# LLNL/parelag

Measured on NVIDIA B200. Metric: vcycle_dofs_per_s, higher is better.
Workload: dtype f64

## Files before the change

include/parelag_b200.h:

```cpp
#ifndef PARELAG_B200_H
#define PARELAG_B200_H

#include <stddef.h>
#include <stdint.h>

#ifdef __cplusplus
extern "C" {
#endif

typedef struct pe_ctx pe_ctx;
typedef struct pe_mat pe_mat;
typedef struct pe_vec pe_vec;
typedef struct pe_smoother pe_smoother;
typedef struct pe_graph pe_graph;

typedef struct pe_parcsr_host {
    int64_t global_num_rows, global_num_cols;
    int64_t first_row_index, first_col_diag;
    int32_t num_rows;
    int32_t num_cols_diag;
    int32_t num_cols_offd;
    const int32_t *diag_i, *diag_j;
    const double *diag_data;
    const int32_t *offd_i, *offd_j;
// ... 17 lines not shown
int pe_ctx_timer_start(pe_ctx *ctx);
int pe_ctx_timer_stop(pe_ctx *ctx, float *ms);
int pe_ctx_profile(pe_ctx *ctx, int enable);
int pe_ctx_profile_get(pe_ctx *ctx, int kernel_id, int64_t *count, double *total_ms, double *total_bytes);
enum { PE_TUNE_SELL_MIN_ROWS = 0, PE_TUNE_SELL_GROUP = 1, PE_TUNE_PDL = 2, PE_TUNE_GATHER_KEEP_PCT = 3, PE_TUNE_P2P_HALO = 4,
       PE_TUNE_FUSED_GS_MAX_MB = 5, PE_TUNE_GS_SLABS = 6, PE_TUNE_LOCAL_SMEM_BYTES = 7, PE_TUNE_COUNT = 8 };
int pe_set_tuning(int key, int value);
int pe_get_tuning(int key);
enum { PE_VARIANT_SPMV_SELL = 0, PE_VARIANT_SPMV_STREAM = 1, PE_VARIANT_SPMV_VECTOR = 2,
       PE_VARIANT_SPGEMM_SYM_T128 = 3, PE_VARIANT_SPGEMM_SYM_T1024 = 4, PE_VARIANT_SPGEMM_SYM_T8192 = 5, PE_VARIANT_SPGEMM_SYM_GMEM = 6,
       PE_VARIANT_SPGEMM_NUM_T128 = 7, PE_VARIANT_SPGEMM_NUM_T1024 = 8, PE_VARIANT_SPGEMM_NUM_T8192 = 9, PE_VARIANT_SPGEMM_NUM_GMEM = 10,
       PE_VARIANT_RELAX_TPR_1 = 11, PE_VARIANT_RELAX_TPR_2 = 12, PE_VARIANT_RELAX_TPR_4 = 13, PE_VARIANT_RELAX_TPR_8 = 14,
       PE_VARIANT_RELAX_TPR_16 = 15, PE_VARIANT_RELAX_TPR_32 = 16,
       PE_VARIANT_TRACES_SMEM = 17, PE_VARIANT_TRACES_GMEM = 18, PE_VARIANT_EXT_SMEM = 19, PE_VARIANT_EXT_GMEM = 20,
       PE_VARIANT_EXT_SPLIT_SMEM = 21, PE_VARIANT_TRACES_GMEM_REUSE = 22, PE_VARIANT_EXT_GMEM_REUSE = 23,
       PE_VARIANT_COUNT = 24 };
int pe_variant_counts(int64_t *out, int n, int reset);
int pe_ctx_flush_l2(pe_ctx *ctx);

int pe_graph_begin(pe_ctx *ctx);
int pe_graph_end(pe_ctx *ctx, pe_graph **out);
int pe_graph_launch(pe_ctx *ctx, pe_graph *g);
int pe_graph_free(pe_graph *g);

typedef struct pe_program pe_program;
int pe_program_begin(pe_ctx *ctx);
int pe_program_end(pe_ctx *ctx, pe_program **out);
int pe_program_launch(pe_ctx *ctx, pe_program *p);
int pe_program_free(pe_program *p);
int pe_program_info(const pe_program *p, int32_t *nops, double *algorithmic_bytes);
int pe_program_profile(pe_ctx *ctx, pe_program *p, int32_t *op_types, double *op_usec, double *op_bytes);
// ... 78 lines not shown
```

parelag_b200/capi.py:

```python
import ctypes as C
import os
import re

import numpy as np

_HERE = os.path.dirname(os.path.abspath(__file__))
LIB_PATH = os.path.join(_HERE, "lib", "libparelag_b200.so")
HEADER_PATHS = [os.path.join(os.path.dirname(_HERE), "include", "parelag_b200_local.h"),
                os.path.join(os.path.dirname(_HERE), "include", "parelag_b200.h"),
                os.path.join(os.path.dirname(_HERE), "include", "parelag_b200_api.h")]

_lib = None


class PEError(RuntimeError):
    pass


class ParCSRHost(C.Structure):
    _fields_ = [
        ("global_num_rows", C.c_int64), ("global_num_cols", C.c_int64),
        ("first_row_index", C.c_int64), ("first_col_diag", C.c_int64),
        ("num_rows", C.c_int32), ("num_cols_diag", C.c_int32), ("num_cols_offd", C.c_int32),
        ("diag_i", C.c_void_p), ("diag_j", C.c_void_p), ("diag_data", C.c_void_p),
# ... 110 lines not shown

def get_tuning(key):
    return lib().pe_get_tuning(key)


REPLAY_DIRECT = 0
REPLAY_GRAPH = 1
REPLAY_PROGRAM = 2
REPLAY_MODE_NAMES = {REPLAY_DIRECT: "direct", REPLAY_GRAPH: "graph", REPLAY_PROGRAM: "program"}

VARIANT_SLOTS = ("SPMV_SELL", "SPMV_STREAM", "SPMV_VECTOR",
                 "SPGEMM_SYM_T128", "SPGEMM_SYM_T1024", "SPGEMM_SYM_T8192", "SPGEMM_SYM_GMEM",
                 "SPGEMM_NUM_T128", "SPGEMM_NUM_T1024", "SPGEMM_NUM_T8192", "SPGEMM_NUM_GMEM",
                 "RELAX_TPR_1", "RELAX_TPR_2", "RELAX_TPR_4", "RELAX_TPR_8", "RELAX_TPR_16", "RELAX_TPR_32",
                 "TRACES_SMEM", "TRACES_GMEM", "EXT_SMEM", "EXT_GMEM",
                 "EXT_SPLIT_SMEM", "TRACES_GMEM_REUSE", "EXT_GMEM_REUSE")
(SPMV_SELL, SPMV_STREAM, SPMV_VECTOR,
 SPGEMM_SYM_T128, SPGEMM_SYM_T1024, SPGEMM_SYM_T8192, SPGEMM_SYM_GMEM,
 SPGEMM_NUM_T128, SPGEMM_NUM_T1024, SPGEMM_NUM_T8192, SPGEMM_NUM_GMEM,
 RELAX_TPR_1, RELAX_TPR_2, RELAX_TPR_4, RELAX_TPR_8, RELAX_TPR_16, RELAX_TPR_32,
 TRACES_SMEM, TRACES_GMEM, EXT_SMEM, EXT_GMEM,
 EXT_SPLIT_SMEM, TRACES_GMEM_REUSE, EXT_GMEM_REUSE) = range(len(VARIANT_SLOTS))


def variant_counts(reset=False):
    out = np.zeros(len(VARIANT_SLOTS), dtype=np.int64)
    _chk(lib().pe_variant_counts(_ptr(out), len(VARIANT_SLOTS), 1 if reset else 0))
    return out


def nccl_unique_id():
    buf = C.create_string_buffer(128)
    _chk(lib().pe_nccl_get_unique_id(buf))
    return buf.raw


class Vec:
# ... 222 lines not shown
```

parelag_b200/csrc/pe_core.cuh:

```cuda
#pragma once
#include <cuda_runtime.h>
#include <stdint.h>
#include <memory>
#include <string>
#include <vector>
#include "../../include/parelag_b200.h"

#define PE_SM_COUNT 148

void pe_set_error(const std::string &msg);

#define PE_CUDA(call)                                                              \
    do {                                                                           \
        cudaError_t e_ = (call);                                                   \
        if (e_ != cudaSuccess) {                                                   \
            pe_set_error(std::string(#call) + " failed: " + cudaGetErrorString(e_) \
                         + " at " + __FILE__ + ":" + std::to_string(__LINE__));    \
            return 1;                                                              \
        }                                                                          \
    } while (0)

#define PE_CHECK(cond, msg)                                     \
    do {                                                        \
        if (!(cond)) {                                          \
// ... 6 lines not shown
    do {                          \
        int rc_ = (expr);         \
        if (rc_) return rc_;      \
    } while (0)

#define PE_LAUNCHED(ctx)                                     \
    do {                                                     \
        (ctx)->launches++;                                   \
        if ((ctx)->rec) pe_rec_fail((ctx), __FILE__, __LINE__); \
        PE_CUDA(cudaPeekAtLastError());                      \
    } while (0)

enum PeOpType : int32_t {
    PE_OP_SELL_SPMV = 1, PE_OP_SELL_GS, PE_OP_CSR_SPMV, PE_OP_PERM_IN, PE_OP_PERM_OUT, PE_OP_AXPBY, PE_OP_ADD3,
    PE_OP_FILL, PE_OP_COPY, PE_OP_SCALE, PE_OP_MUL, PE_OP_DOT, PE_OP_DOT_FIN, PE_OP_AXPY_DEV, PE_OP_XPBY_DEV,
    PE_OP_PCG_STEP
};
struct PeOp {
    int32_t type, i0, i1, i2, i3, i4, i5, flags;
    int64_t n;
    double a, b;
    const void *p[9];
};
struct pe_recorder {
    std::vector<PeOp> ops;
    std::vector<double> bytes;
    bool failed = false;
    std::string why;
};
struct pe_ctx;
void pe_rec_fail(pe_ctx *ctx, const char *file, int line);
// ... 60 lines not shown
    }
    return cudaLaunchKernelEx(&cfg, kern, KArgs(args)...);
}
#endif
int pe_prof_begin(pe_ctx *ctx, int id, double bytes);
int pe_prof_end(pe_ctx *ctx);
#define PE_MAX_PARTIALS 4096

struct DevSELL {
    int32_t nslices = 0, nrows = 0;
    int32_t wmax = 0;
    int64_t nstored = 0;
    int32_t *soff = nullptr;
    int32_t *J = nullptr;
    double *A = nullptr;
};

struct DevCSR {
    int32_t nrows = 0, ncols = 0;
    int64_t nnz = 0;
    int32_t *I = nullptr, *J = nullptr;
    double *A = nullptr;
    int32_t *rb = nullptr;
    int32_t nrb = 0;
    DevSELL *sell = nullptr;
    int sell_state = 0;
};
void pe_sell_free(DevSELL &m);
int pe_sell_build(pe_ctx *ctx, const DevCSR &diag, const DevCSR *offd, const int32_t *rowmap_d, int32_t nslices,
                  const int32_t *colpos_d, int32_t ext_base, DevSELL &out,
                  std::vector<int32_t> *soff_host = nullptr);
int pe_sell_for_spmv(pe_ctx *ctx, DevCSR &m);
void pe_mat_values_changed(struct pe_mat *A);
int pe_launch_sell_spmv(pe_ctx *ctx, const DevSELL &S, double alpha, const double *x, double beta,
                        const double *yin, double *yout);
int pe_launch_sell_gs(pe_ctx *ctx, const DevSELL &S, int s0, int s1, int wmax, int ext_base, const double *f, double *u,
                      const double *uext, const double *l1, uint64_t pol_gather);
int pe_make_gather_policy(pe_ctx *ctx, int keep_pct, uint64_t *pol);
int pe_launch_perm_in(pe_ctx *ctx, int n, const int *pos, const double *b, const double *x, double *fp, double *up);
int pe_launch_perm_out(pe_ctx *ctx, int n, const int *pos, const double *up, double *x);
#define PE_STREAM_NNZ 2048
#define PE_STREAM_CAP 2560
#define PE_STREAM_MAXROW 512
int pe_build_row_blocks(pe_ctx *ctx, DevCSR &m, const std::vector<int32_t> *forced_breaks);
int devcsr_alloc(DevCSR &m, int32_t nrows, int32_t ncols, int64_t nnz);
void devcsr_free(DevCSR &m);

struct pe_vec {
    pe_ctx *ctx;
    int64_t n;
    double *d;
    bool view = false;
};

struct pe_mat {
// ... 54 lines not shown
```

parelag_b200/csrc/pe_prog.cu:

```cuda
#include "pe_core.cuh"
#include "pe_stream.cuh"
#include <cstring>

#define PROG_THREADS 1024
#define PROG_WARPS (PROG_THREADS / 32)

struct pe_program {
    pe_ctx *ctx = nullptr;
    PeOp *ops_d = nullptr;
    int nops = 0, grid = 0;
    unsigned long long *bar_d = nullptr;
    unsigned long long epoch = 0;
    unsigned long long *ts_d = nullptr;
    std::vector<int32_t> types;
    std::vector<double> bytes;
    double total_bytes = 0.0;
};

__device__ __forceinline__ unsigned long long ld_acquire_u64(const unsigned long long *p)
{
    unsigned long long v;
    asm volatile("ld.acquire.gpu.global.u64 %0, [%1];" : "=l"(v) : "l"(p) : "memory");
    return v;
}
__device__ __forceinline__ unsigned long long globaltimer_ns()
{
    unsigned long long t;
    asm volatile("mov.u64 %0, %globaltimer;" : "=l"(t));
    return t;
}

__device__ __noinline__ void op_sell_spmv(const PeOp &o, int gw, int W, int lane)
{
    const int nslices = o.i0, nrows = o.i1;
    const int *soff = (const int *)o.p[0], *J = (const int *)o.p[1];
    const double *A = (const double *)o.p[2], *x = (const double *)o.p[3], *yin = (const double *)o.p[4];
    double *yout = (double *)o.p[5];
    const double alpha = o.a, beta = o.b;
    const uint64_t pol = l2_evict_first_policy();
    for (int s = gw; s < nslices; s += W)
    {
        const int o0 = __ldg(soff + s), w = __ldg(soff + s + 1) - o0;
        const int *j = J + (int64_t)o0 * 32 + lane;
        const double *a = A + (int64_t)o0 * 32 + lane;
        double acc = 0.0;
        int q = 0;
        for (; q + 4 <= w; q += 4)
        {
            const int c0 = ld_stream_s32(j + (q + 0) * 32, pol), c1 = ld_stream_s32(j + (q + 1) * 32, pol);
            const int c2 = ld_stream_s32(j + (q + 2) * 32, pol), c3 = ld_stream_s32(j + (q + 3) * 32, pol);
            const double a0 = ld_stream_f64(a + (q + 0) * 32, pol), a1 = ld_stream_f64(a + (q + 1) * 32, pol);
            const double a2 = ld_stream_f64(a + (q + 2) * 32, pol), a3 = ld_stream_f64(a + (q + 3) * 32, pol);
            const double x0 = __ldcg(x + c0), x1 = __ldcg(x + c1), x2 = __ldcg(x + c2), x3 = __ldcg(x + c3);
            acc += a0 * x0; acc += a1 * x1; acc += a2 * x2; acc += a3 * x3;
        }
        for (; q < w; ++q) acc += ld_stream_f64(a + q * 32, pol) * __ldcg(x + ld_stream_s32(j + q * 32, pol));
        const int row = s * 32 + lane;
        if (row < nrows)
        {
            double v = alpha * acc;
            if (beta != 0.0) v += beta * __ldcg(yin + row);
            yout[row] = v;
        }
    }
}

__device__ __noinline__ void op_sell_gs(const PeOp &o, int gw, int W, int lane)
{
    const int s0 = o.i0, s1 = o.i1, ext_base = o.i2;
    const int *soff = (const int *)o.p[0], *J = (const int *)o.p[1];
    const double *A = (const double *)o.p[2], *f = (const double *)o.p[3];
    double *u = (double *)o.p[4];
    const double *uext = (const double *)o.p[5], *l1 = (const double *)o.p[6];
    const uint64_t pol = l2_evict_first_policy();
#define PE_GATHER(c) ((uext && (c) >= ext_base) ? __ldcg(uext + ((c) - ext_base)) : __ldcg(u + (c)))
    for (int s = s0 + gw; s < s1; s += W)
    {
        const int o0 = __ldg(soff + s), w = __ldg(soff + s + 1) - o0;
        const int *j = J + (int64_t)o0 * 32 + lane;
// ... 70 lines not shown
    }
}

__device__ __noinline__ void op_elementwise(const PeOp &o, int64_t gt, int64_t T)
{
    const int64_t n = o.n;
    const double a = o.a, b = o.b;
    switch (o.type)
    {
    case PE_OP_PERM_IN:
    {
        const int *pos = (const int *)o.p[0];
        const double *bv = (const double *)o.p[1], *x = (const double *)o.p[2];
        double *fp = (double *)o.p[3], *up = (double *)o.p[4];
        for (int64_t i = gt; i < n; i += T) { const int p = __ldg(pos + i); fp[p] = __ldcg(bv + i); up[p] = x ? __ldcg(x + i) : 0.0; }
        break;
    }
    case PE_OP_PERM_OUT:
    {
        const int *pos = (const int *)o.p[0];
        const double *up = (const double *)o.p[1];
        double *x = (double *)o.p[2];
        for (int64_t i = gt; i < n; i += T) x[i] = __ldcg(up + __ldg(pos + i));
        break;
    }
    case PE_OP_AXPBY:
    {
        const double *x = (const double *)o.p[0];
        double *y = (double *)o.p[1];
        if (b == 0.0) { for (int64_t i = gt; i < n; i += T) y[i] = a * __ldcg(x + i); }
// ... 248 lines not shown
```

parelag_b200/csrc/pe_relax.cu:

```cuda
#include "pe_core.cuh"
#include "pe_stream.cuh"
#include <algorithm>
#include <cmath>
#include <cstring>

struct pe_smoother {
    pe_ctx *ctx = nullptr;
    pe_mat *A = nullptr;
    int type = 2, sweeps = 1, cheby_order = 2, ordering = 0;
    double weight = 1.0, omega = 1.0, cheby_fraction = 0.3;
    double *l1_d = nullptr;
    double *v_d = nullptr, *w_d = nullptr, *z_d = nullptr, *r_d = nullptr;
    int32_t nsets = 0;
    std::vector<int32_t> set_starts;
    std::vector<int32_t> order;
    int32_t *perm_d = nullptr;
    DevCSR P;
    uint8_t *before_d = nullptr;
    int tpr = 8;
    std::vector<int> set_pI;
    std::vector<int> set_rb;
    int pI_at(int k) const { for (size_t c = 0; c < set_starts.size(); ++c) if (set_starts[c] == k) return set_pI[c]; return 0; }
    bool use_sell = false;
    DevSELL S;
// ... 889 lines not shown
extern "C" int pe_smoother_apply(pe_smoother *s, const pe_vec *b, pe_vec *x, int iterative_mode)
{
    pe_ctx *ctx = s->ctx;
    pe_mat *A = s->A;
    int n = A->diag.nrows;
    PE_CHECK(b->n == n && x->n == n, "pe_smoother_apply: size mismatch");
    cudaStream_t st = ctx->stream;
    if (s->use_sell)
    {
        const bool ghosts = A->offd.nnz > 0;
        for (int sweep = 0; sweep < s->sweeps; ++sweep)
        {
            const bool zero_guess = !iterative_mode && sweep == 0;
            PE_TRY(sweep_halo(A, x->d, zero_guess));
            if (s->fused && !ctx->rec) { PE_TRY(launch_fused_sweep(s, b->d, x->d, zero_guess)); continue; }
            PE_TRY(pe_launch_perm_in(ctx, n, s->pos_d, b->d, zero_guess ? nullptr : x->d, s->fp_d, s->up_d));
            for (int pass = 0; pass < 2; ++pass)
                for (int cc = (pass == 1 && s->skip_turn) ? 1 : 0; cc < s->nsets; ++cc)
                {
                    const int c = pass == 0 ? cc : s->nsets - 1 - cc;
                    if (s->slice_starts[c + 1] == s->slice_starts[c]) continue;
                    PE_TRY(pe_prof_begin(ctx, s->set_bytes[c] >= 64e6 ? 1 : 3, s->set_bytes[c]));
                    PE_TRY(pe_launch_sell_gs(ctx, s->S, s->slice_starts[c], s->slice_starts[c + 1], s->set_wmax[c], s->npad, s->fp_d, s->up_d,
                                             ghosts ? A->x_ext_d : nullptr, s->l1p_d, s->pol_gather));
                    PE_TRY(pe_prof_end(ctx));
                }
            PE_TRY(pe_launch_perm_out(ctx, n, s->pos_d, s->up_d, x->d));
        }
        return 0;
    }
    if (!iterative_mode) PE_CUDA(cudaMemsetAsync(x->d, 0, sizeof(double) * (size_t)n, st));
    const int *oI = A->offd.nnz > 0 ? A->offd.I : nullptr;
    for (int sweep = 0; sweep < s->sweeps; ++sweep) {
        if (s->type == 0 || s->type == 1 || s->type == 5) {
            PE_TRY(sweep_halo(A, x->d, !iterative_mode && sweep == 0));
            int tpr = A->tpr;
// ... 68 lines not shown
```

parelag_b200/csrc/pe_sell.cu:

```cuda
#include "pe_core.cuh"
#include "pe_stream.cuh"
#include <cub/cub.cuh>
#include <algorithm>

__device__ __forceinline__ int sell_src_row(const int *rowmap, int k, int nrows_src)
{
    if (rowmap) return rowmap[k];
    return k < nrows_src ? k : -1;
}

__global__ void k_sell_widths(int nslices, int nrows_src, const int *__restrict__ rowmap,
                              const int *__restrict__ dI, const int *__restrict__ oI, int *w)
{
    const int s = (blockIdx.x * blockDim.x + threadIdx.x) >> 5, lane = threadIdx.x & 31;
    if (s >= nslices) return;
    const int r = sell_src_row(rowmap, s * 32 + lane, nrows_src);
    int len = 0;
    if (r >= 0) { len = dI[r + 1] - dI[r]; if (oI) len += oI[r + 1] - oI[r]; }
    len = __reduce_max_sync(0xffffffffu, len);
    if (lane == 0) { w[s + 1] = len; if (s == 0) w[0] = 0; }
}

__global__ void k_sell_fill(int nslices, int nrows_src, const int *__restrict__ rowmap,
                            const int *__restrict__ colpos, int ext_base,
// ... 16 lines not shown
        }
        if (oI) for (int t = oI[r]; t < oI[r + 1]; ++t, ++q, p += 32)
        {
            last = ext_base + oJ[t];
            J[p] = last; A[p] = oA[t];
        }
    }
    for (; q < w; ++q, p += 32) { J[p] = last; A[p] = 0.0; }
}

void pe_sell_free(DevSELL &m)
{
    if (m.soff) cudaFree(m.soff);
    if (m.J) cudaFree(m.J);
    if (m.A) cudaFree(m.A);
    m = DevSELL();
}

int pe_sell_build(pe_ctx *ctx, const DevCSR &diag, const DevCSR *offd, const int32_t *rowmap_d, int32_t nslices,
                  const int32_t *colpos_d, int32_t ext_base, DevSELL &out, std::vector<int32_t> *soff_host)
{
    cudaStream_t st = ctx->stream;
    if (!rowmap_d) nslices = (diag.nrows + 31) / 32;
    out = DevSELL();
    out.nslices = nslices;
    out.nrows = diag.nrows;
    PE_CUDA(cudaMalloc(&out.soff, sizeof(int32_t) * (size_t)(nslices + 1)));
    if (nslices == 0) { PE_CUDA(cudaMemsetAsync(out.soff, 0, sizeof(int32_t), st)); return 0; }
    const int *oI = (offd && offd->nnz > 0) ? offd->I : nullptr;
    const int grid = pe_grid_for((int64_t)nslices * 32, 256);
// ... 12 lines not shown
    out.wmax = 0;
    for (int32_t k = 0; k < nslices; ++k) out.wmax = std::max(out.wmax, soff_h[k + 1] - soff_h[k]);
    if (soff_host) soff_host->swap(soff_h);
    out.nstored = (int64_t)total * 32;
    PE_CUDA(cudaMalloc(&out.J, sizeof(int32_t) * (size_t)(out.nstored > 0 ? out.nstored : 1)));
    PE_CUDA(cudaMalloc(&out.A, sizeof(double) * (size_t)(out.nstored > 0 ? out.nstored : 1)));
    if (out.nstored > 0)
    {
        k_sell_fill<<<grid, 256, 0, st>>>(nslices, diag.nrows, rowmap_d, colpos_d, ext_base, diag.I, diag.J, diag.A,
                                          oI, oI ? offd->J : nullptr, oI ? offd->A : nullptr, out.soff, out.J, out.A);
        PE_LAUNCHED(ctx);
    }
    return 0;
}

int pe_sell_for_spmv(pe_ctx *ctx, DevCSR &m)
{
    if (m.sell_state != 0) return 0;
    m.sell_state = -1;
    if (m.nnz == 0 || m.nrows == 0) return 0;
    DevSELL *s = new DevSELL();
    int rc = pe_sell_build(ctx, m, nullptr, nullptr, 0, nullptr, 0, *s);
    if (rc) { delete s; return rc; }
    if ((double)s->nstored > 1.25 * (double)m.nnz) { pe_sell_free(*s); delete s; return 0; }
    m.sell = s;
    m.sell_state = 1;
    return 0;
}

template <int G, bool PRO = false>
__device__ __forceinline__ void sell_load_group(const int *j, const double *a, int q, int w, uint64_t pol,
                                                int (&c)[G], double (&v)[G])
{
#pragma unroll
    for (int k = 0; k < G; ++k)
        if (q + k < w)
        {
            c[k] = PRO ? ld_stream_s32_pro(j + (q + k) * 32, pol) : ld_stream_s32(j + (q + k) * 32, pol);
            v[k] = PRO ? ld_stream_f64_pro(a + (q + k) * 32, pol) : ld_stream_f64(a + (q + k) * 32, pol);
        }
}

template <int G>
__device__ __forceinline__ void sell_pin_group_then_wait(const int (&c)[G], const double (&v)[G], int w)
{
    int t = 0;
#pragma unroll
    for (int k = 0; k < G; ++k) if (k < w) t ^= c[k] ^ __double2hiint(v[k]) ^ __double2loint(v[k]);
    if (t == 0x5bd1e995) pdl_trigger();
    pdl_wait();
}

template <int G, bool SINGLE>
__global__ void __launch_bounds__(256, ((SINGLE || G <= 4) ? 4 : 2))
k_sell_spmv(int nslices, int nrows, const int *__restrict__ soff, const int *__restrict__ J,
            const double *__restrict__ A, const double *x, double alpha, double beta,
            const double *yin, double *yout)
{
    pdl_trigger();
    const int s = (blockIdx.x * blockDim.x + threadIdx.x) >> 5, lane = threadIdx.x & 31;
    if (s >= nslices) { pdl_wait(); return; }
    const int o0 = ld_nc_s32_pro(soff + s), w = ld_nc_s32_pro(soff + s + 1) - o0;
    const int *j = J + (int64_t)o0 * 32 + lane;
    const double *a = A + (int64_t)o0 * 32 + lane;
    const uint64_t pol = l2_evict_first_policy();
    double acc = 0.0;
    int c[G]; double v[G];
    sell_load_group<G, true>(j, a, 0, w, pol, c, v);
    sell_pin_group_then_wait<G>(c, v, w);
    const int row = s * 32 + lane;
    const double yv = (beta != 0.0 && row < nrows) ? yin[row] : 0.0;
    for (int q = 0; q < w; q += G)
    {
        double xv[G], b[G];
#pragma unroll
        for (int k = 0; k < G; ++k) if (q + k < w) { xv[k] = x[c[k]]; b[k] = v[k]; }
        if (!SINGLE && q + G < w) sell_load_group<G>(j, a, q + G, w, pol, c, v);
#pragma unroll
        for (int k = 0; k < G; ++k) if (q + k < w) acc = __fma_rn(b[k], xv[k], acc);
// ... 47 lines not shown
    else if (wmax <= 4) G = 4;
    else if (wmax <= 8) G = 8;
    else if (wmax <= 12) G = 12;
    else if (wmax <= 24) G = 8;
    else G = 4;
    single = wmax <= G;
}

int pe_launch_sell_spmv(pe_ctx *ctx, const DevSELL &S, double alpha, const double *x, double beta,
                        const double *yin, double *yout)
{
    if (S.nslices == 0) return 0;
    if (ctx->rec)
    {
        PeOp o = pe_op(PE_OP_SELL_SPMV); o.i0 = S.nslices; o.i1 = S.nrows; o.a = alpha; o.b = beta;
        o.p[0] = S.soff; o.p[1] = S.J; o.p[2] = S.A; o.p[3] = x; o.p[4] = yin; o.p[5] = yout;
        pe_rec_push(ctx, o, -1.0);
        return 0;
    }
    const int grid = pe_grid_for((int64_t)S.nslices * 32, 256);
    int G; bool single;
    sell_pick_group(S.wmax, G, single);
#define PE_SPMV(GG, SS) PE_CUDA(pe_launch_k(ctx, k_sell_spmv<GG, SS>, grid, 256, S.nslices, S.nrows, S.soff, S.J, S.A, x, alpha, beta, yin, yout))
    if (G == 4) { if (single) PE_SPMV(4, true); else PE_SPMV(4, false); }
    else if (G == 8) { if (single) PE_SPMV(8, true); else PE_SPMV(8, false); }
    else { if (single) PE_SPMV(12, true); else PE_SPMV(12, false); }
#undef PE_SPMV
    PE_LAUNCHED(ctx);
    return 0;
}

template <int G, bool SINGLE, bool OFFD>
__global__ void __launch_bounds__(256, ((SINGLE || G <= 4) ? 4 : 2))
k_sell_gs(int s0, int s1, const int *__restrict__ soff, const int *__restrict__ J, const double *__restrict__ A,
          int ext_base, const double *f, double *u, const double *uext,
          const double *__restrict__ l1, uint64_t pol_u)
{
    pdl_trigger();
    const int s = s0 + ((blockIdx.x * blockDim.x + threadIdx.x) >> 5), lane = threadIdx.x & 31;
    if (s >= s1) { pdl_wait(); return; }
    const int o0 = ld_nc_s32_pro(soff + s), w = ld_nc_s32_pro(soff + s + 1) - o0;
    const int *j = J + (int64_t)o0 * 32 + lane;
// ... 66 lines not shown
    if (i < n) x[i] = up[p];
}
int pe_launch_perm_in(pe_ctx *ctx, int n, const int *pos, const double *b, const double *x, double *fp, double *up)
{
    if (n == 0) return 0;
    if (ctx->rec)
    {
        PeOp o = pe_op(PE_OP_PERM_IN); o.n = n; o.p[0] = pos; o.p[1] = b; o.p[2] = x; o.p[3] = fp; o.p[4] = up;
        pe_rec_push(ctx, o, 0.0);
        return 0;
    }
    PE_CUDA(pe_launch_k(ctx, k_sell_perm_in, pe_grid_for(n, 256), 256, n, pos, b, x, fp, up));
    PE_LAUNCHED(ctx);
    return 0;
}
int pe_launch_perm_out(pe_ctx *ctx, int n, const int *pos, const double *up, double *x)
{
    if (n == 0) return 0;
    if (ctx->rec)
    {
        PeOp o = pe_op(PE_OP_PERM_OUT); o.n = n; o.p[0] = pos; o.p[1] = up; o.p[2] = x;
        pe_rec_push(ctx, o, 0.0);
        return 0;
    }
    PE_CUDA(pe_launch_k(ctx, k_sell_perm_out, pe_grid_for(n, 256), 256, n, pos, up, x));
    PE_LAUNCHED(ctx);
    return 0;
}
```

parelag_b200/csrc/pe_spmv.cu:

```cuda
#include "pe_core.cuh"
#include <cub/cub.cuh>

__device__ __forceinline__ double ld_stream_f64(const double *p)
{
    double v;
    asm volatile("ld.global.nc.L1::no_allocate.f64 %0, [%1];" : "=d"(v) : "l"(p));
    return v;
}
__device__ __forceinline__ int ld_stream_s32(const int *p)
{
    int v;
    asm volatile("ld.global.nc.L1::no_allocate.s32 %0, [%1];" : "=r"(v) : "l"(p));
    return v;
}

template <int TPR>
__global__ void __launch_bounds__(256)
k_spmv(int n, const int *__restrict__ dI, const int *__restrict__ dJ, const double *__restrict__ dA,
       const int *__restrict__ oI, const int *__restrict__ oJ, const double *__restrict__ oA,
       const double *x, const double *xext,
       double alpha, double beta, const double *yin, double *yout)
{
    pdl_trigger();
    const int lane = threadIdx.x & (TPR - 1);
// ... 62 lines not shown
}

int pe_launch_spmv(pe_ctx *ctx, const DevCSR &diag, const DevCSR *offd, int tpr,
                   double alpha, const double *x, const double *xext,
                   double beta, const double *yin, double *yout)
{
    int n = diag.nrows;
    if (n == 0) return 0;
    const int *oI = nullptr, *oJ = nullptr;
    const double *oA = nullptr;
    if (offd && offd->nnz > 0) { oI = offd->I; oJ = offd->J; oA = offd->A; }
    if (!oI && diag.sell_state == 0) PE_TRY(pe_sell_for_spmv(ctx, const_cast<DevCSR &>(diag)));
    if (!oI && diag.sell)
    {
        pe_variant_add(PE_VARIANT_SPMV_SELL, n);
        PE_TRY(pe_prof_begin(ctx, 0, 12.0 * (double)diag.nnz + 4.0 * (n + 1) + 8.0 * diag.ncols + 8.0 * n + (beta != 0.0 ? 8.0 * n : 0.0)));
        PE_TRY(pe_launch_sell_spmv(ctx, *diag.sell, alpha, x, beta, yin, yout));
        PE_TRY(pe_prof_end(ctx));
        return 0;
    }
    if (ctx->rec && !oI)
    {
        pe_variant_add(PE_VARIANT_SPMV_VECTOR, n);
        PeOp o = pe_op(PE_OP_CSR_SPMV); o.i0 = n; o.i1 = pe_choose_tpr(diag.nnz, n); o.a = alpha; o.b = beta;
        o.p[0] = diag.I; o.p[1] = diag.J; o.p[2] = diag.A; o.p[3] = x; o.p[4] = yin; o.p[5] = yout;
        pe_rec_push(ctx, o, 12.0 * (double)diag.nnz + 4.0 * (n + 1) + 8.0 * diag.ncols + 8.0 * n + (beta != 0.0 ? 8.0 * n : 0.0));
        return 0;
    }
    if (!oI && diag.nrb == 0 && diag.nnz > 0) PE_TRY(pe_build_row_blocks(ctx, const_cast<DevCSR &>(diag), nullptr));
    if (!oI && diag.nrb > 0)
    {
// ... 203 lines not shown
```

parelag_b200/csrc/pe_stream.cuh:

```cuda
#pragma once
#include <stdint.h>
#include "../../include/parelag_b200.h"

__device__ __forceinline__ uint64_t l2_evict_first_policy()
{
    uint64_t pol;
    asm("createpolicy.fractional.L2::evict_first.b64 %0, 1.0;" : "=l"(pol));
    return pol;
}
__device__ __forceinline__ double ld_stream_f64(const double *p, uint64_t pol)
{
    double v;
    asm("ld.global.nc.L1::no_allocate.L2::cache_hint.f64 %0, [%1], %2;" : "=d"(v) : "l"(p), "l"(pol));
    return v;
}
__device__ __forceinline__ int ld_stream_s32(const int *p, uint64_t pol)
{
    int v;
    asm("ld.global.nc.L1::no_allocate.L2::cache_hint.s32 %0, [%1], %2;" : "=r"(v) : "l"(p), "l"(pol));
    return v;
}

__device__ __forceinline__ double ld_stream_f64_pro(const double *p, uint64_t pol)
{
    double v;
    asm volatile("ld.global.nc.L1::no_allocate.L2::cache_hint.f64 %0, [%1], %2;" : "=d"(v) : "l"(p), "l"(pol));
    return v;
}
__device__ __forceinline__ int ld_stream_s32_pro(const int *p, uint64_t pol)
{
    int v;
    asm volatile("ld.global.nc.L1::no_allocate.L2::cache_hint.s32 %0, [%1], %2;" : "=r"(v) : "l"(p), "l"(pol));
    return v;
}
__device__ __forceinline__ int ld_nc_s32_pro(const int *p)
{
    int v;
    asm volatile("ld.global.nc.s32 %0, [%1];" : "=r"(v) : "l"(p));
    return v;
}
__device__ __forceinline__ double ld_nc_f64_pro(const double *p)
{
    double v;
    asm volatile("ld.global.nc.f64 %0, [%1];" : "=d"(v) : "l"(p));
    return v;
}

__device__ __forceinline__ void pe_pcg_scalar_step_dev(double *s, int phase, int iter, int max_iter, double rel, double abs_tol)
// ... 47 lines not shown
```

parelag_b200/src/parelag_solvers.hpp:

```cpp
#pragma once
#include <algorithm>
#include <cctype>
#include <cmath>
#include <cstdio>
#include "parelag_core.hpp"
#include "parelag_sequence.hpp"
#include "parelag_block.hpp"

namespace parelag
{

namespace mg_utils
{
inline void ComputeResidual(const mfem::Operator &A, const mfem::Vector &x, const mfem::Vector &b, mfem::Vector &r)
{
    auto A_hyp = dynamic_cast<const mfem::HypreParMatrix *>(&A);
    if (!A_hyp) { ComputeResidualGeneric(A, x, b, r); return; }
    r.SetSize(b.Size());
    PE_CALL(pe_residual(Device::Get(), A_hyp->Handle(), x.Read(), b.Read(), r.Write()));
}
}

inline bool SolverCaptureSafe(const mfem::Solver *s)
{
// ... 97 lines not shown
    {
        PARELAG_ASSERT(A_); PARELAG_ASSERT(D_op_); PARELAG_ASSERT(PrimarySolver_); PARELAG_ASSERT(AuxiliarySolver_);
        AuxB_.SetSize(D_op_->Width());
        AuxX_.SetSize(D_op_->Width());
        PrimaryVec_.SetSize(A_->Height());
    }
    void Mult(const mfem::Vector &B, mfem::Vector &X) const override
    {
        if (this->IsPreconditioner()) X = 0.0;
        PARELAG_ASSERT(PrimarySolver_->iterative_mode);
        PrimarySolver_->Mult(B, X);
        mg_utils::ComputeResidual(*A_, X, B, PrimaryVec_);
        D_op_->MultTranspose(PrimaryVec_, AuxB_);
        PARELAG_ASSERT(!AuxiliarySolver_->iterative_mode);
        AuxiliarySolver_->Mult(AuxB_, AuxX_);
        D_op_->Mult(AuxX_, PrimaryVec_);
        X += PrimaryVec_;
    }
    void MultTranspose(const mfem::Vector &B, mfem::Vector &X) const override
    {
        if (this->IsPreconditioner()) { X = 0.0; D_op_->MultTranspose(B, AuxB_); }
        else { mg_utils::ComputeResidual(*A_, X, B, PrimaryVec_); D_op_->MultTranspose(PrimaryVec_, AuxB_); }
        AuxiliarySolver_->Mult(AuxB_, AuxX_);
        D_op_->Mult(AuxX_, PrimaryVec_);
        X += PrimaryVec_;
        PrimarySolver_->Mult(B, X);
    }
    Op_Ptr GetAuxiliaryOperator() const { return A_aux_; }
    bool CaptureSafe() const override
    { return SolverCaptureSafe(PrimarySolver_.get()) && SolverCaptureSafe(AuxiliarySolver_.get()); }
private:
    void _do_set_operator(const Op_Ptr &) override { PARELAG_NOT_IMPLEMENTED(); }
    Op_Ptr A_, A_aux_, D_op_;
    std::shared_ptr<mfem::Solver> PrimarySolver_, AuxiliarySolver_;
    mutable mfem::Vector AuxB_, AuxX_, PrimaryVec_;
};

class HiptmairSmootherFactory : public SolverFactory
{
public:
    explicit HiptmairSmootherFactory(const ParameterList &params = ParameterList()) { SetParameters(params); }
    explicit HiptmairSmootherFactory(std::shared_ptr<SolverFactory> SmootherFact, const ParameterList &params = ParameterList())
        : PrimaryFact_(std::move(SmootherFact)), AuxiliaryFact_(PrimaryFact_) { SetParameters(params); }
    HiptmairSmootherFactory(std::shared_ptr<SolverFactory> PrimarySolverFactory, std::shared_ptr<SolverFactory> AuxiliarySolverFactory,
                            const ParameterList &params = ParameterList())
        : PrimaryFact_(std::move(PrimarySolverFactory)), AuxiliaryFact_(std::move(AuxiliarySolverFactory)) { SetParameters(params); }
// ... 1010 lines not shown
```

Baseline: 1.214 billion.

## Encode ±1 SELL matrices as int8, fuse first GS color into perm-in, fuse aux correction

When a SELL matrix used for SpMV holds only the values 0 and ±1, the values are stored as int8 signs and the double array is freed, so each nonzero streams 5 bytes instead of 12. The zero-guess Gauss-Seidel sweep now folds the first colour set into the permute-in kernel, because with a zero initial guess that set's update is just b/l1, which saves one GS launch. The Hiptmair smoother adds the auxiliary correction with a single y = Dx + y SpMV on one rank instead of an SpMV followed by a separate vector add. The costs are an extra detection kernel and a host sync when the SELL format is built.

```diff
diff --git a/include/parelag_b200.h b/include/parelag_b200.h
--- a/include/parelag_b200.h
+++ b/include/parelag_b200.h
@@ -55,7 +55,7 @@
        PE_VARIANT_RELAX_TPR_16 = 15, PE_VARIANT_RELAX_TPR_32 = 16,
        PE_VARIANT_TRACES_SMEM = 17, PE_VARIANT_TRACES_GMEM = 18, PE_VARIANT_EXT_SMEM = 19, PE_VARIANT_EXT_GMEM = 20,
        PE_VARIANT_EXT_SPLIT_SMEM = 21, PE_VARIANT_TRACES_GMEM_REUSE = 22, PE_VARIANT_EXT_GMEM_REUSE = 23,
-       PE_VARIANT_COUNT = 24 };
+       PE_VARIANT_SPMV_SELL_SIGNS = 24, PE_VARIANT_COUNT = 25 };
 int pe_variant_counts(int64_t *out, int n, int reset);
 int pe_ctx_flush_l2(pe_ctx *ctx);
 
diff --git a/parelag_b200/capi.py b/parelag_b200/capi.py
--- a/parelag_b200/capi.py
+++ b/parelag_b200/capi.py
@@ -148,13 +148,13 @@
                  "SPGEMM_NUM_T128", "SPGEMM_NUM_T1024", "SPGEMM_NUM_T8192", "SPGEMM_NUM_GMEM",
                  "RELAX_TPR_1", "RELAX_TPR_2", "RELAX_TPR_4", "RELAX_TPR_8", "RELAX_TPR_16", "RELAX_TPR_32",
                  "TRACES_SMEM", "TRACES_GMEM", "EXT_SMEM", "EXT_GMEM",
-                 "EXT_SPLIT_SMEM", "TRACES_GMEM_REUSE", "EXT_GMEM_REUSE")
+                 "EXT_SPLIT_SMEM", "TRACES_GMEM_REUSE", "EXT_GMEM_REUSE", "SPMV_SELL_SIGNS")
 (SPMV_SELL, SPMV_STREAM, SPMV_VECTOR,
  SPGEMM_SYM_T128, SPGEMM_SYM_T1024, SPGEMM_SYM_T8192, SPGEMM_SYM_GMEM,
  SPGEMM_NUM_T128, SPGEMM_NUM_T1024, SPGEMM_NUM_T8192, SPGEMM_NUM_GMEM,
  RELAX_TPR_1, RELAX_TPR_2, RELAX_TPR_4, RELAX_TPR_8, RELAX_TPR_16, RELAX_TPR_32,
  TRACES_SMEM, TRACES_GMEM, EXT_SMEM, EXT_GMEM,
- EXT_SPLIT_SMEM, TRACES_GMEM_REUSE, EXT_GMEM_REUSE) = range(len(VARIANT_SLOTS))
+ EXT_SPLIT_SMEM, TRACES_GMEM_REUSE, EXT_GMEM_REUSE, SPMV_SELL_SIGNS) = range(len(VARIANT_SLOTS))
 
 
 def variant_counts(reset=False):
diff --git a/parelag_b200/csrc/pe_core.cuh b/parelag_b200/csrc/pe_core.cuh
--- a/parelag_b200/csrc/pe_core.cuh
+++ b/parelag_b200/csrc/pe_core.cuh
@@ -44,7 +44,7 @@
 enum PeOpType : int32_t {
     PE_OP_SELL_SPMV = 1, PE_OP_SELL_GS, PE_OP_CSR_SPMV, PE_OP_PERM_IN, PE_OP_PERM_OUT, PE_OP_AXPBY, PE_OP_ADD3,
     PE_OP_FILL, PE_OP_COPY, PE_OP_SCALE, PE_OP_MUL, PE_OP_DOT, PE_OP_DOT_FIN, PE_OP_AXPY_DEV, PE_OP_XPBY_DEV,
-    PE_OP_PCG_STEP
+    PE_OP_PCG_STEP, PE_OP_PERM_IN_GS0
 };
 struct PeOp {
     int32_t type, i0, i1, i2, i3, i4, i5, flags;
@@ -135,6 +135,7 @@
     int32_t *soff = nullptr;
     int32_t *J = nullptr;
     double *A = nullptr;
+    int8_t *S = nullptr;
 };
 
 struct DevCSR {
@@ -160,6 +161,8 @@
 int pe_make_gather_policy(pe_ctx *ctx, int keep_pct, uint64_t *pol);
 int pe_launch_perm_in(pe_ctx *ctx, int n, const int *pos, const double *b, const double *x, double *fp, double *up);
 int pe_launch_perm_out(pe_ctx *ctx, int n, const int *pos, const double *up, double *x);
+int pe_launch_perm_in_gs0(pe_ctx *ctx, int n, const int *pos, const double *b, int r0, int r1, const double *l1,
+                          double *fp, double *up);
 #define PE_STREAM_NNZ 2048
 #define PE_STREAM_CAP 2560
 #define PE_STREAM_MAXROW 512
diff --git a/parelag_b200/csrc/pe_prog.cu b/parelag_b200/csrc/pe_prog.cu
--- a/parelag_b200/csrc/pe_prog.cu
+++ b/parelag_b200/csrc/pe_prog.cu
@@ -30,11 +30,15 @@
     return t;
 }
 
-__device__ __noinline__ void op_sell_spmv(const PeOp &o, int gw, int W, int lane)
+__device__ __forceinline__ double op_ld_value(const double *a, uint64_t pol) { return ld_stream_f64(a, pol); }
+__device__ __forceinline__ double op_ld_value(const int8_t *a, uint64_t pol) { return ld_stream_s8(a, pol); }
+
+template <typename V>
+__device__ __forceinline__ void sell_spmv_body(const PeOp &o, const V *A, int gw, int W, int lane)
 {
     const int nslices = o.i0, nrows = o.i1;
     const int *soff = (const int *)o.p[0], *J = (const int *)o.p[1];
-    const double *A = (const double *)o.p[2], *x = (const double *)o.p[3], *yin = (const double *)o.p[4];
+    const double *x = (const double *)o.p[3], *yin = (const double *)o.p[4];
     double *yout = (double *)o.p[5];
     const double alpha = o.a, beta = o.b;
     const uint64_t pol = l2_evict_first_policy();
@@ -42,19 +46,19 @@
     {
         const int o0 = __ldg(soff + s), w = __ldg(soff + s + 1) - o0;
         const int *j = J + (int64_t)o0 * 32 + lane;
-        const double *a = A + (int64_t)o0 * 32 + lane;
+        const V *a = A + (int64_t)o0 * 32 + lane;
         double acc = 0.0;
         int q = 0;
         for (; q + 4 <= w; q += 4)
         {
             const int c0 = ld_stream_s32(j + (q + 0) * 32, pol), c1 = ld_stream_s32(j + (q + 1) * 32, pol);
             const int c2 = ld_stream_s32(j + (q + 2) * 32, pol), c3 = ld_stream_s32(j + (q + 3) * 32, pol);
-            const double a0 = ld_stream_f64(a + (q + 0) * 32, pol), a1 = ld_stream_f64(a + (q + 1) * 32, pol);
-            const double a2 = ld_stream_f64(a + (q + 2) * 32, pol), a3 = ld_stream_f64(a + (q + 3) * 32, pol);
+            const double a0 = op_ld_value(a + (q + 0) * 32, pol), a1 = op_ld_value(a + (q + 1) * 32, pol);
+            const double a2 = op_ld_value(a + (q + 2) * 32, pol), a3 = op_ld_value(a + (q + 3) * 32, pol);
             const double x0 = __ldcg(x + c0), x1 = __ldcg(x + c1), x2 = __ldcg(x + c2), x3 = __ldcg(x + c3);
             acc += a0 * x0; acc += a1 * x1; acc += a2 * x2; acc += a3 * x3;
         }
-        for (; q < w; ++q) acc += ld_stream_f64(a + q * 32, pol) * __ldcg(x + ld_stream_s32(j + q * 32, pol));
+        for (; q < w; ++q) acc += op_ld_value(a + q * 32, pol) * __ldcg(x + ld_stream_s32(j + q * 32, pol));
         const int row = s * 32 + lane;
         if (row < nrows)
         {
@@ -63,6 +67,11 @@
             yout[row] = v;
         }
     }
+}
+__device__ __noinline__ void op_sell_spmv(const PeOp &o, int gw, int W, int lane)
+{
+    if (o.p[6]) sell_spmv_body(o, (const int8_t *)o.p[6], gw, W, lane);
+    else sell_spmv_body(o, (const double *)o.p[2], gw, W, lane);
 }
 
 __device__ __noinline__ void op_sell_gs(const PeOp &o, int gw, int W, int lane)
@@ -163,6 +172,21 @@
         const double *bv = (const double *)o.p[1], *x = (const double *)o.p[2];
         double *fp = (double *)o.p[3], *up = (double *)o.p[4];
         for (int64_t i = gt; i < n; i += T) { const int p = __ldg(pos + i); fp[p] = __ldcg(bv + i); up[p] = x ? __ldcg(x + i) : 0.0; }
+        break;
+    }
+    case PE_OP_PERM_IN_GS0:
+    {
+        const int *pos = (const int *)o.p[0];
+        const double *bv = (const double *)o.p[1], *l1 = (const double *)o.p[2];
+        double *fp = (double *)o.p[3], *up = (double *)o.p[4];
+        for (int64_t i = gt; i < n; i += T)
+        {
+            const int p = __ldg(pos + i);
+            const double d = (p >= o.i0 && p < o.i1) ? __ldcg(l1 + p) : 0.0;
+            const double fr = __ldcg(bv + i), ur = 0.0, acc = 0.0;
+            fp[p] = fr;
+            up[p] = d != 0.0 ? ur + (fr - acc) / d : ur;
+        }
         break;
     }
     case PE_OP_PERM_OUT:
diff --git a/parelag_b200/csrc/pe_relax.cu b/parelag_b200/csrc/pe_relax.cu
--- a/parelag_b200/csrc/pe_relax.cu
+++ b/parelag_b200/csrc/pe_relax.cu
@@ -927,12 +927,20 @@
             const bool zero_guess = !iterative_mode && sweep == 0;
             PE_TRY(sweep_halo(A, x->d, zero_guess));
             if (s->fused && !ctx->rec) { PE_TRY(launch_fused_sweep(s, b->d, x->d, zero_guess)); continue; }
-            PE_TRY(pe_launch_perm_in(ctx, n, s->pos_d, b->d, zero_guess ? nullptr : x->d, s->fp_d, s->up_d));
+            int first = -1;
+            if (zero_guess && s->nsets > 0)
+            {
+                first = 0;
+                while (first < s->nsets - 1 && s->slice_starts[first + 1] == s->slice_starts[first]) ++first;
+                PE_TRY(pe_launch_perm_in_gs0(ctx, n, s->pos_d, b->d, 32 * s->slice_starts[first], 32 * s->slice_starts[first + 1],
+                                             s->l1p_d, s->fp_d, s->up_d));
+            }
+            else PE_TRY(pe_launch_perm_in(ctx, n, s->pos_d, b->d, zero_guess ? nullptr : x->d, s->fp_d, s->up_d));
             for (int pass = 0; pass < 2; ++pass)
                 for (int cc = (pass == 1 && s->skip_turn) ? 1 : 0; cc < s->nsets; ++cc)
                 {
                     const int c = pass == 0 ? cc : s->nsets - 1 - cc;
-                    if (s->slice_starts[c + 1] == s->slice_starts[c]) continue;
+                    if (s->slice_starts[c + 1] == s->slice_starts[c] || (pass == 0 && c == first)) continue;
                     PE_TRY(pe_prof_begin(ctx, s->set_bytes[c] >= 64e6 ? 1 : 3, s->set_bytes[c]));
                     PE_TRY(pe_launch_sell_gs(ctx, s->S, s->slice_starts[c], s->slice_starts[c + 1], s->set_wmax[c], s->npad, s->fp_d, s->up_d,
                                              ghosts ? A->x_ext_d : nullptr, s->l1p_d, s->pol_gather));
diff --git a/parelag_b200/csrc/pe_sell.cu b/parelag_b200/csrc/pe_sell.cu
--- a/parelag_b200/csrc/pe_sell.cu
+++ b/parelag_b200/csrc/pe_sell.cu
@@ -54,6 +54,7 @@
     if (m.soff) cudaFree(m.soff);
     if (m.J) cudaFree(m.J);
     if (m.A) cudaFree(m.A);
+    if (m.S) cudaFree(m.S);
     m = DevSELL();
 }
 
@@ -96,6 +97,34 @@
     return 0;
 }
 
+__global__ void k_sell_signs(int64_t n, const double *__restrict__ A, int8_t *S, int *bad)
+{
+    const int64_t i = (int64_t)blockIdx.x * blockDim.x + threadIdx.x;
+    if (i >= n) return;
+    const double v = A[i];
+    const int8_t c = v == 1.0 ? 1 : (v == -1.0 ? -1 : 0);
+    if (c == 0 && v != 0.0) *bad = 1;
+    S[i] = c;
+}
+
+static int sell_encode_signs(pe_ctx *ctx, DevSELL &s)
+{
+    if (s.nstored == 0) return 0;
+    cudaStream_t st = ctx->stream;
+    int *bad_d = nullptr, bad = 0;
+    PE_CUDA(cudaMalloc(&s.S, (size_t)s.nstored));
+    PE_CUDA(cudaMalloc(&bad_d, sizeof(int)));
+    PE_CUDA(cudaMemsetAsync(bad_d, 0, sizeof(int), st));
+    k_sell_signs<<<pe_grid_for(s.nstored, 256), 256, 0, st>>>(s.nstored, s.A, s.S, bad_d);
+    PE_LAUNCHED(ctx);
+    PE_CUDA(cudaMemcpyAsync(&bad, bad_d, sizeof(int), cudaMemcpyDeviceToHost, st));
+    PE_CUDA(cudaStreamSynchronize(st));
+    cudaFree(bad_d);
+    if (bad) { cudaFree(s.S); s.S = nullptr; }
+    else { cudaFree(s.A); s.A = nullptr; }
+    return 0;
+}
+
 int pe_sell_for_spmv(pe_ctx *ctx, DevCSR &m)
 {
     if (m.sell_state != 0) return 0;
@@ -105,13 +134,22 @@
     int rc = pe_sell_build(ctx, m, nullptr, nullptr, 0, nullptr, 0, *s);
     if (rc) { delete s; return rc; }
     if ((double)s->nstored > 1.25 * (double)m.nnz) { pe_sell_free(*s); delete s; return 0; }
+    rc = sell_encode_signs(ctx, *s);
+    if (rc) { pe_sell_free(*s); delete s; return rc; }
     m.sell = s;
     m.sell_state = 1;
     return 0;
 }
 
-template <int G, bool PRO = false>
-__device__ __forceinline__ void sell_load_group(const int *j, const double *a, int q, int w, uint64_t pol,
+template <bool PRO>
+__device__ __forceinline__ double sell_load_value(const double *a, uint64_t pol)
+{ return PRO ? ld_stream_f64_pro(a, pol) : ld_stream_f64(a, pol); }
+template <bool PRO>
+__device__ __forceinline__ double sell_load_value(const int8_t *a, uint64_t pol)
+{ return PRO ? ld_stream_s8_pro(a, pol) : ld_stream_s8(a, pol); }
+
+template <int G, bool PRO = false, typename V>
+__device__ __forceinline__ void sell_load_group(const int *j, const V *a, int q, int w, uint64_t pol,
                                                 int (&c)[G], double (&v)[G])
 {
 #pragma unroll
@@ -119,7 +157,7 @@
         if (q + k < w)
         {
             c[k] = PRO ? ld_stream_s32_pro(j + (q + k) * 32, pol) : ld_stream_s32(j + (q + k) * 32, pol);
-            v[k] = PRO ? ld_stream_f64_pro(a + (q + k) * 32, pol) : ld_stream_f64(a + (q + k) * 32, pol);
+            v[k] = sell_load_value<PRO>(a + (q + k) * 32, pol);
         }
 }
 
@@ -133,10 +171,10 @@
     pdl_wait();
 }
 
-template <int G, bool SINGLE>
+template <int G, bool SINGLE, typename V>
 __global__ void __launch_bounds__(256, ((SINGLE || G <= 4) ? 4 : 2))
 k_sell_spmv(int nslices, int nrows, const int *__restrict__ soff, const int *__restrict__ J,
-            const double *__restrict__ A, const double *x, double alpha, double beta,
+            const V *__restrict__ A, const double *x, double alpha, double beta,
             const double *yin, double *yout)
 {
     pdl_trigger();
@@ -144,7 +182,7 @@
     if (s >= nslices) { pdl_wait(); return; }
     const int o0 = ld_nc_s32_pro(soff + s), w = ld_nc_s32_pro(soff + s + 1) - o0;
     const int *j = J + (int64_t)o0 * 32 + lane;
-    const double *a = A + (int64_t)o0 * 32 + lane;
+    const V *a = A + (int64_t)o0 * 32 + lane;
     const uint64_t pol = l2_evict_first_policy();
     double acc = 0.0;
     int c[G]; double v[G];
@@ -222,18 +260,20 @@
     if (ctx->rec)
     {
         PeOp o = pe_op(PE_OP_SELL_SPMV); o.i0 = S.nslices; o.i1 = S.nrows; o.a = alpha; o.b = beta;
-        o.p[0] = S.soff; o.p[1] = S.J; o.p[2] = S.A; o.p[3] = x; o.p[4] = yin; o.p[5] = yout;
+        o.p[0] = S.soff; o.p[1] = S.J; o.p[2] = S.A; o.p[3] = x; o.p[4] = yin; o.p[5] = yout; o.p[6] = S.S;
         pe_rec_push(ctx, o, -1.0);
         return 0;
     }
     const int grid = pe_grid_for((int64_t)S.nslices * 32, 256);
     int G; bool single;
     sell_pick_group(S.wmax, G, single);
-#define PE_SPMV(GG, SS) PE_CUDA(pe_launch_k(ctx, k_sell_spmv<GG, SS>, grid, 256, S.nslices, S.nrows, S.soff, S.J, S.A, x, alpha, beta, yin, yout))
+#define PE_SPMV_V(GG, SS, VV, AA) PE_CUDA(pe_launch_k(ctx, k_sell_spmv<GG, SS, VV>, grid, 256, S.nslices, S.nrows, S.soff, S.J, AA, x, alpha, beta, yin, yout))
+#define PE_SPMV(GG, SS) do { if (S.S) PE_SPMV_V(GG, SS, int8_t, (const int8_t *)S.S); else PE_SPMV_V(GG, SS, double, (const double *)S.A); } while (0)
     if (G == 4) { if (single) PE_SPMV(4, true); else PE_SPMV(4, false); }
     else if (G == 8) { if (single) PE_SPMV(8, true); else PE_SPMV(8, false); }
     else { if (single) PE_SPMV(12, true); else PE_SPMV(12, false); }
 #undef PE_SPMV
+#undef PE_SPMV_V
     PE_LAUNCHED(ctx);
     return 0;
 }
@@ -330,6 +370,35 @@
     PE_LAUNCHED(ctx);
     return 0;
 }
+
+__global__ void k_sell_perm_in_gs0(int n, const int *__restrict__ pos, const double *b, int r0, int r1,
+                                   const double *__restrict__ l1, double *fp, double *up)
+{
+    pdl_trigger();
+    const int i = blockIdx.x * blockDim.x + threadIdx.x;
+    const int p = i < n ? pos[i] : 0;
+    const double d = (i < n && p >= r0 && p < r1) ? l1[p] : 0.0;
+    pdl_wait();
+    if (i >= n) return;
+    const double fr = b[i], ur = 0.0, acc = 0.0;
+    fp[p] = fr;
+    up[p] = d != 0.0 ? ur + (fr - acc) / d : ur;
+}
+int pe_launch_perm_in_gs0(pe_ctx *ctx, int n, const int *pos, const double *b, int r0, int r1, const double *l1,
+                          double *fp, double *up)
+{
+    if (n == 0) return 0;
+    if (ctx->rec)
+    {
+        PeOp o = pe_op(PE_OP_PERM_IN_GS0); o.n = n; o.i0 = r0; o.i1 = r1;
+        o.p[0] = pos; o.p[1] = b; o.p[2] = l1; o.p[3] = fp; o.p[4] = up;
+        pe_rec_push(ctx, o, 0.0);
+        return 0;
+    }
+    PE_CUDA(pe_launch_k(ctx, k_sell_perm_in_gs0, pe_grid_for(n, 256), 256, n, pos, b, r0, r1, l1, fp, up));
+    PE_LAUNCHED(ctx);
+    return 0;
+}
 int pe_launch_perm_out(pe_ctx *ctx, int n, const int *pos, const double *up, double *x)
 {
     if (n == 0) return 0;
diff --git a/parelag_b200/csrc/pe_spmv.cu b/parelag_b200/csrc/pe_spmv.cu
--- a/parelag_b200/csrc/pe_spmv.cu
+++ b/parelag_b200/csrc/pe_spmv.cu
@@ -100,7 +100,9 @@
     if (!oI && diag.sell)
     {
         pe_variant_add(PE_VARIANT_SPMV_SELL, n);
-        PE_TRY(pe_prof_begin(ctx, 0, 12.0 * (double)diag.nnz + 4.0 * (n + 1) + 8.0 * diag.ncols + 8.0 * n + (beta != 0.0 ? 8.0 * n : 0.0)));
+        if (diag.sell->S) pe_variant_add(PE_VARIANT_SPMV_SELL_SIGNS, n);
+        const double per_nnz = diag.sell->S ? 5.0 : 12.0;
+        PE_TRY(pe_prof_begin(ctx, 0, per_nnz * (double)diag.nnz + 4.0 * (n + 1) + 8.0 * diag.ncols + 8.0 * n + (beta != 0.0 ? 8.0 * n : 0.0)));
         PE_TRY(pe_launch_sell_spmv(ctx, *diag.sell, alpha, x, beta, yin, yout));
         PE_TRY(pe_prof_end(ctx));
         return 0;
diff --git a/parelag_b200/csrc/pe_stream.cuh b/parelag_b200/csrc/pe_stream.cuh
--- a/parelag_b200/csrc/pe_stream.cuh
+++ b/parelag_b200/csrc/pe_stream.cuh
@@ -32,6 +32,18 @@
     int v;
     asm volatile("ld.global.nc.L1::no_allocate.L2::cache_hint.s32 %0, [%1], %2;" : "=r"(v) : "l"(p), "l"(pol));
     return v;
+}
+__device__ __forceinline__ double ld_stream_s8(const int8_t *p, uint64_t pol)
+{
+    int v;
+    asm("ld.global.nc.L1::no_allocate.L2::cache_hint.s8 %0, [%1], %2;" : "=r"(v) : "l"(p), "l"(pol));
+    return (double)v;
+}
+__device__ __forceinline__ double ld_stream_s8_pro(const int8_t *p, uint64_t pol)
+{
+    int v;
+    asm volatile("ld.global.nc.L1::no_allocate.L2::cache_hint.s8 %0, [%1], %2;" : "=r"(v) : "l"(p), "l"(pol));
+    return (double)v;
 }
 __device__ __forceinline__ int ld_nc_s32_pro(const int *p)
 {
diff --git a/parelag_b200/src/parelag_solvers.hpp b/parelag_b200/src/parelag_solvers.hpp
--- a/parelag_b200/src/parelag_solvers.hpp
+++ b/parelag_b200/src/parelag_solvers.hpp
@@ -135,22 +135,27 @@
         D_op_->MultTranspose(PrimaryVec_, AuxB_);
         PARELAG_ASSERT(!AuxiliarySolver_->iterative_mode);
         AuxiliarySolver_->Mult(AuxB_, AuxX_);
-        D_op_->Mult(AuxX_, PrimaryVec_);
-        X += PrimaryVec_;
+        AddAuxiliaryCorrection(X);
     }
     void MultTranspose(const mfem::Vector &B, mfem::Vector &X) const override
     {
         if (this->IsPreconditioner()) { X = 0.0; D_op_->MultTranspose(B, AuxB_); }
         else { mg_utils::ComputeResidual(*A_, X, B, PrimaryVec_); D_op_->MultTranspose(PrimaryVec_, AuxB_); }
         AuxiliarySolver_->Mult(AuxB_, AuxX_);
-        D_op_->Mult(AuxX_, PrimaryVec_);
-        X += PrimaryVec_;
+        AddAuxiliaryCorrection(X);
         PrimarySolver_->Mult(B, X);
     }
     Op_Ptr GetAuxiliaryOperator() const { return A_aux_; }
     bool CaptureSafe() const override
     { return SolverCaptureSafe(PrimarySolver_.get()) && SolverCaptureSafe(AuxiliarySolver_.get()); }
 private:
+    void AddAuxiliaryCorrection(mfem::Vector &X) const
+    {
+        auto D_hyp = dynamic_cast<const mfem::HypreParMatrix *>(D_op_.get());
+        if (D_hyp && pe_ctx_nranks(Device::Get()) == 1) { D_hyp->Mult(1.0, AuxX_, 1.0, X); return; }
+        D_op_->Mult(AuxX_, PrimaryVec_);
+        X += PrimaryVec_;
+    }
     void _do_set_operator(const Op_Ptr &) override { PARELAG_NOT_IMPLEMENTED(); }
     Op_Ptr A_, A_aux_, D_op_;
     std::shared_ptr<mfem::Solver> PrimarySolver_, AuxiliarySolver_;
```

New measurement: 1.252 billion (median of 6 runs). 1.03x the previous value.
